# yangao07/LAMSA

Hardware: AMD Instinct MI355X
Metric: aligned Gbase/s, 10 kbp ONT-error reads (12%: sub/ins/del 4% each), -T ont2d vs GRCh37-sized stand-in; inputs resident in HBM when the timed region starts (upload excluded: see pcie_inclusive_*) (higher is better)
Workload: dtype int32

## Files before the change

### lamsa_amd/csrc/hp_core.h

```cpp
#pragma once
#include <hp/wave.h>
#include "../../include/lamsa_hp.h"

namespace hp {

typedef int32_t cig_t;
enum { C_M = 0, C_I = 1, C_D = 2, C_N = 3, C_S = 4, C_H = 5, C_EQ = 7, C_X = 8 };
enum { ST_OVERFLOW = LAMSA_HP_ST_OVERFLOW, ST_REFEXIT = LAMSA_HP_ST_REFEXIT, ST_UNSUPPORTED = LAMSA_HP_ST_UNSUPPORTED,
       ST_DEAD = ST_OVERFLOW | ST_REFEXIT | ST_UNSUPPORTED };

#define HP_NEG_INF (-0x40000000)

struct Arena {
    char *base; size_t cap, top;
};
HP_INL void arena_init(Arena &a, void *base, size_t cap) { a.base = (char *)base; a.cap = cap; a.top = 0; }
HP_INL size_t arena_mark(const Arena &a) { return a.top; }
HP_INL void arena_release(Arena &a, size_t m) { a.top = m; }

#ifndef HP_LDS_CELLS
#define HP_LDS_CELLS 512
#endif
#ifndef HP_LDS_Z_BYTES
#define HP_LDS_Z_BYTES 512
#endif
#define HP_LDS_WORDS (2 * HP_LDS_CELLS + HP_LDS_CELLS / 4 + HP_LDS_Z_BYTES / 4)
#ifndef HP_CHAIN_LDS_WORDS
#define HP_CHAIN_LDS_WORDS 2432
#endif
#define HP_BOTH_LDS_WORDS (HP_CHAIN_LDS_WORDS > HP_LDS_WORDS ? HP_CHAIN_LDS_WORDS : HP_LDS_WORDS)
#define HP_LANE_STRIP_WORDS HP_CHAIN_LDS_WORDS

struct Ctx {
    const lamsa_hp_para *P;
    HP_L int32_t *lds;
    int lds_words;
    Arena tmp;
    int status;
    long long n_cells;
    long long *prof;
    long long *prof_dp = nullptr;
    int lds_epoch;
};
#if defined(HP_PROF_EDGE) && (defined(HP_PROF_TRACK) || defined(HP_PROF_FILL))
#error "-DHP_PROF_EDGE, -DHP_PROF_TRACK and -DHP_PROF_FILL all use prof slots 16 .. 23: one of them per build"
#endif
#ifdef HP_PROF_FILL
#define HP_PROF_CHAIN_ON 0
#define HP_TADD_FILL(cx, slot, v) HP_TADD(cx, slot, v)
#else
#define HP_PROF_CHAIN_ON 1
#define HP_TADD_FILL(cx, slot, v) do { } while (0)
#endif
#ifdef HP_PROF
#define HP_T0(v) const long long v = wv::clock()
#define HP_TADD(cx, slot, v) do { if ((cx).prof) { (cx).prof[slot] += wv::clock() - (v); (cx).prof[(slot) + 1] += 1; } } while (0)
#else
#define HP_T0(v) do { } while (0)
#define HP_TADD(cx, slot, v) do { } while (0)
#endif

#ifndef HP_DPLOG
#define HP_DPLOG(kind, qlen, tlen, w, cells) do { } while (0)
#endif
#ifndef HP_STAT
#define HP_STAT(i) do { } while (0)
#endif
#ifndef HP_STAT_ADD
#define HP_STAT_ADD(i, n) ((void)0)
#endif
#ifndef HP_STAT_MAX
#define HP_STAT_MAX(i, v) ((void)0)
#endif
#ifdef HP_STAT_SLOTS
static_assert(HP_STAT_SLOTS >= 92, "the array of the path counters ends before the last slot the device sources use");
#define HP_STATX_ADD(i, n) HP_STAT_ADD(i, n)
#define HP_STATX_MAX(i, v) HP_STAT_MAX(i, v)
#else
#define HP_STATX_ADD(i, n) ((void)0)
#define HP_STATX_MAX(i, v) ((void)0)
#endif

HP_INL void *arena_alloc(Ctx &cx, size_t bytes) {
    size_t b = (bytes + 15) & ~(size_t)15;
    if (cx.tmp.top + b > cx.tmp.cap) { cx.status |= ST_OVERFLOW; return nullptr; }
    void *p = cx.tmp.base + cx.tmp.top;
    cx.tmp.top += b;
    return p;
}

struct CigV { cig_t *c; int n, cap; };
HP_INL void cig_bind(CigV &v, cig_t *mem, int cap) { v.c = mem; v.n = 0; v.cap = mem ? cap : 0; }
HP_INL bool cig_alloc(Ctx &cx, CigV &v, int cap) {
    cig_t *m = (cig_t *)arena_alloc(cx, (size_t)cap * sizeof(cig_t));
    cig_bind(v, m, cap);
    return m != nullptr;
}
HP_INL void cig_raw_push(Ctx &cx, CigV &v, cig_t w) {
    if (v.n >= v.cap) { cx.status |= ST_OVERFLOW; return; }
    v.c[v.n++] = w;
}
HP_INL void cig_push0(Ctx &cx, CigV &v, cig_t w) {
    if (v.n > 0 && (v.c[v.n - 1] & 0xf) == (w & 0xf)) { v.c[v.n - 1] += (w >> 4) << 4; return; }
    cig_raw_push(cx, v, w);
}
HP_INL void cig_push1(Ctx &cx, CigV &v, cig_t w) { if ((w >> 4) == 0) return; cig_push0(cx, v, w); }
HP_FN void cig_pushv(Ctx &cx, CigV &v, const cig_t *c, int n) {
    if (n == 0) return;
    const HP_G cig_t *src = (const HP_G cig_t *)c;
    HP_G cig_t *dst = (HP_G cig_t *)v.c;
    const int vn = v.n;
    int j = 0;
    if (vn > 0) {
        const cig_t last = dst[vn - 1], c0 = src[0];
        if ((last & 0xf) == (c0 & 0xf)) { dst[vn - 1] = last + ((c0 >> 4) << 4); j = 1; }
        else if (((last & 0xf) == C_I && (c0 & 0xf) == C_S) || ((last & 0xf) == C_S && (c0 & 0xf) == C_I)) {
            dst[vn - 1] = (((last >> 4) + (c0 >> 4)) << 4) | C_S; j = 1;
        }
    }
    const int m = n - j;
    if (vn + m > v.cap) { cx.status |= ST_OVERFLOW; return; }
    for (int b0 = 0; b0 < m; b0 += 64) { WAVE_FOR(l) { const int i = b0 + l; if (i < m) dst[vn + i] = src[j + i]; } }
    v.n = vn + m;
    wv::sync();
}
HP_FN void cig_pushw(Ctx &cx, CigV &v, cig_t w) {
    if (v.n > 0) {
        const cig_t last = v.c[v.n - 1];
        if ((last & 0xf) == (w & 0xf)) { v.c[v.n - 1] = last + ((w >> 4) << 4); return; }
        if (((last & 0xf) == C_I && (w & 0xf) == C_S) || ((last & 0xf) == C_S && (w & 0xf) == C_I)) { v.c[v.n - 1] = (((last >> 4) + (w >> 4)) << 4) | C_S; return; }
    }
    if (v.n + 1 > v.cap) { cx.status |= ST_OVERFLOW; return; }
    v.c[v.n++] = w;
}
HP_FN void cig_invert(cig_t *c, int n) {
    HP_G cig_t *g = (HP_G cig_t *)c;
    for (int b0 = 0; b0 < n / 2; b0 += 64) {
        WAVE_FOR(l) { const int a = b0 + l; if (a < n / 2) { const cig_t x = g[a], y = g[n - 1 - a]; g[a] = y; g[n - 1 - a] = x; } }
    }
    wv::sync();
}
HP_FN int cig_readlen(const cig_t *c, int n) {
    const HP_G cig_t *g = (const HP_G cig_t *)c;
    int tot = 0;
    for (int b0 = 0; b0 < n; b0 += 64) {
        wv::Lane<int> x;
        WAVE_FOR(l) { const int i = b0 + l; int v = 0; if (i < n) { const cig_t w = g[i]; const int op = w & 0xf; if (op == C_M || op == C_I || op == C_S) v = w >> 4; } x[l] = v; }
        tot += wv::reduce_sum(x);
    }
    return tot;
}
HP_FN int cig_reflen(const cig_t *c, int n) {
    const HP_G cig_t *g = (const HP_G cig_t *)c;
    int tot = 0;
    for (int b0 = 0; b0 < n; b0 += 64) {
        wv::Lane<int> x;
        WAVE_FOR(l) { const int i = b0 + l; int v = 0; if (i < n) { const cig_t w = g[i]; const int op = w & 0xf; if (op == C_M || op == C_D || op == C_H) v = w >> 4; } x[l] = v; }
        tot += wv::reduce_sum(x);
    }
    return tot;
}

struct Seq { const uint8_t *p; int stride; };
HP_INL int seq_at(const Seq &s, int i) { return s.p[(long)i * s.stride]; }
HP_INL Seq seq_fwd(const uint8_t *p) { Seq s; s.p = p; s.stride = 1; return s; }
HP_INL Seq seq_rev(const uint8_t *p, int len) { Seq s; s.p = p + (len > 0 ? len - 1 : 0); s.stride = -1; return s; }

HP_INL int sub_score(const lamsa_hp_para *P, int t, int q) { return (t > 3 || q > 3) ? -1 : (t == q ? P->match : -P->mis); }

HP_INL int iabs(int x) { return x < 0 ? -x : x; }
HP_INL int imin(int a, int b) { return a < b ? a : b; }
HP_INL int imax(int a, int b) { return a > b ? a : b; }

}
```

### lamsa_amd/csrc/hp_ksw.h

```cpp
#pragma once
#include "hp_core.h"

namespace hp {

#define HP_ZSTRIDE(n_col) ((((n_col) + 7) >> 3) << 2)
HP_INL size_t z_cap(const Ctx &cx) { const int w = cx.lds_words - (2 * HP_LDS_CELLS + HP_LDS_CELLS / 4); return w > 0 ? (size_t)w * 4 : 0; }
HP_INL size_t z_cap_pk(const Ctx &cx) { return cx.lds_words > 0 ? (size_t)cx.lds_words * 4 : 0; }
#define HP_ZFITS(n_col, rows) ((size_t)HP_ZSTRIDE(n_col) * (size_t)(rows) <= z_cap(cx))
HP_INL int z_nibble(int dir) { return (dir & 3) | ((dir >> 2) & 1) << 2 | ((dir >> 5) & 1) << 3; }
HP_INL void z_row_clear(HP_L uint8_t *LZ, int row, int n_col) {
    HP_L int *p = (HP_L int *)(LZ + row * HP_ZSTRIDE(n_col));
    const int nd = HP_ZSTRIDE(n_col) >> 2;
    for (int d0 = 0; d0 < nd; d0 += 64) { WAVE_FOR(l) { if (d0 + l < nd) p[d0 + l] = -1; } }
}
HP_INL void z_put(HP_L uint8_t *LZ, int row, int n_col, int c, int dir) {
    HP_L int *p = (HP_L int *)(LZ + row * HP_ZSTRIDE(n_col)) + (c >> 3);
    wv::lds_and(p, (int)~((unsigned)(~z_nibble(dir) & 0xf) << ((c & 7) << 2)));
}

HP_FN void dp_backtrack(Ctx &cx, const HP_L uint8_t *lz, const uint8_t *z, const int32_t *rowb, int n_col, int w, int i, int k, CigV &out, int pk_stride = 0)
{
    pk_stride = wv::uni(pk_stride);
    const bool in_lds = z == nullptr;
    const HP_G uint8_t *gz = (const HP_G uint8_t *)wv::uni64((long long)z);
// ... 551 lines not shown
            wv::scan_max_excl(key, HP_SCAN_IDENT);
            WAVE_FOR(l) {
                hcur[l] = -1;
                if (l >= beg && l < end) {
                    int f = 0 - (l - beg) * e_ins;
                    if (l > beg) { const int g = key[l] - (l - 1) * e_ins; f = g > f ? g : f; }
                    int M = m[l], ee = Es[l], h, tt;
                    int dir = M > ee ? 0 : 1; h = M > ee ? M : ee;
                    dir = h > f ? dir : 2;    h = h > f ? h : f;
                    tt = M - oe_del; tt = tt > 0 ? tt : 0; ee -= e_del;
                    if (ee > tt) dir |= 1 << 2; else ee = tt;
                    tt = M - oe_ins; tt = tt > 0 ? tt : 0; f -= e_ins;
                    if (f > tt) dir |= 2 << 4;
                    Es[l] = ee;
                    hcur[l] = h;
                    if (zl) z_put(LZ, i, n_col, l - d_beg, dir); else gz[(long)i * n_col + (l - d_beg)] = (uint8_t)dir;
                }
            }
            int mrow = 0, mj = -1;
            {
                const int hmax = wv::reduce_max(hcur);
                if (hmax >= 0) {
                    wv::Lane<int> eq;
                    WAVE_FOR(l) eq[l] = hcur[l] == hmax;
                    mrow = hmax; mj = 63 - __builtin_clzll(wv::ballot(eq));
                }
            }
            const int h_last = beg < end ? wv::bcast(hcur, end - 1) : h1_init;
            WAVE_FOR(l) { if (hcur[l] < 0) hcur[l] = 0; }
            wv::shr1(hcur, 0);
            wv::Lane<int> nz;
            WAVE_FOR(l) {
                if (beg < end) { if (l == beg) Hs[l] = h1_init; else if (l > beg && l <= end) Hs[l] = hcur[l]; }
                else if (l == end) Hs[l] = h1_init;
                if (l == end) Es[l] = 0;
                nz[l] = l >= beg && l <= end && (Hs[l] != 0 || Es[l] != 0);
            }
            const int jj = beg < end ? end : beg;
            if (jj == qlen) {
                max_ie = gscore > h_last ? max_ie : i;
                gscore = gscore > h_last ? gscore : h_last;
            }
            if (mrow == 0) { stop_rows = true; break; }
            if (mrow > max) { max = mrow; max_i = i; max_j = mj; }
            else if (zdrop > 0) {
                if (i - max_i > mj - max_j) { if (max - mrow - ((i - max_i) - (mj - max_j)) * e_del > zdrop) { stop_rows = true; break; } }
                else { if (max - mrow - ((mj - max_j) - (i - max_i)) * e_ins > zdrop) { stop_rows = true; break; } }
            }
            {
                const unsigned long long nzm = wv::ballot(nz);
                const unsigned long long lowm = nzm & (end < 64 ? ((1ull << end) - 1) : ~0ull);
                const int nb = lowm ? __builtin_ctzll(lowm) : end;
                const unsigned long long upm = nzm & ~((1ull << nb) - 1);
                const int jl = upm ? 63 - __builtin_clzll(upm) : nb - 1;
                beg = nb;
                end = jl + 2 < qlen ? jl + 2 : qlen;
            }
        }
    }
    int i, k;
    if (gscore <= 0 || gscore <= max - end_bonus) { i = max_i; k = max_j; }
    else { i = max_ie; k = qlen - 1; }
    er.qle = k + 1; er.tle = i + 1; er.score = max;
    if (out) { wv::sync(); HP_T0(tb0_); dp_backtrack(cx, zl ? LZ : nullptr, z, rowb, n_col, w, i, k, *out); HP_TADD(cx, 28, tb0_); }
    cx.n_cells += cells_;
    arena_release(cx.tmp, mark);
    HP_TADD(cx, 26, te0_);
#ifdef HP_PROF
    HP_TADD(cx, 60, te0_);
#endif
    return er;
}

#define HP_REGN_SETS 4
#define HP_REGN_QMAX(ns) (64 * (ns) - 2)
HP_INL unsigned long long lt_mask64(int x) { return x <= 0 ? 0ull : (x >= 64 ? ~0ull : ((1ull << x) - 1)); }
template <int NS>
HP_NOINL ExtRes ksw_extend_regn(Ctx &cx, int qlen, Seq q, int tlen, Seq t, int w, int h0, CigV *out)
{
    long long cells_ = 0;
    ExtRes er; er.score = 0; er.qle = 0; er.tle = 0;
    HP_T0(te0_);
    qlen = wv::uni(qlen); tlen = wv::uni(tlen); w = wv::uni(w); h0 = wv::uni(h0);
    const lamsa_hp_para *P = cx.P;
    const int o_ins = wv::uni(P->ins_ext_o), e_ins = wv::uni(P->ins_ext_e), o_del = wv::uni(P->del_ext_o), e_del = wv::uni(P->del_ext_e);
    const int end_bonus = wv::uni(P->end_bonus), zdrop = wv::uni(P->zdrop);
    const int oe_del = o_del + e_del, oe_ins = o_ins + e_ins;
    const int n_col = qlen < 2 * w + 1 ? qlen : 2 * w + 1;
    const size_t mark = arena_mark(cx.tmp);
    const bool zl = HP_ZFITS(n_col, tlen);
    uint8_t *z = zl ? nullptr : (uint8_t *)arena_alloc(cx, (size_t)n_col * tlen + 1);
    int32_t *rowb = zl ? nullptr : (int32_t *)arena_alloc(cx, sizeof(int32_t) * 2 * ((size_t)tlen + 1));
    if (!zl && (!z || !rowb)) { arena_release(cx.tmp, mark); return er; }
#ifdef HP_PROF
    if (!zl && cx.prof) { cx.prof[52] += (long long)n_col * tlen; cx.prof[53] += 1; }
#endif
    HP_L uint8_t *LZ = (HP_L uint8_t *)(cx.lds + 2 * HP_LDS_CELLS) + HP_LDS_CELLS;
    HP_G uint8_t *gz = (HP_G uint8_t *)wv::uni64((long long)z);
    HP_G int32_t *growb = (HP_G int32_t *)wv::uni64((long long)rowb);
    const int sc_match = wv::uni(P->match), sc_mis = -wv::uni(P->mis);
    const HP_G uint8_t *gq = (const HP_G uint8_t *)wv::uni64((long long)q.p); const int qs = wv::uni(q.stride);
    const HP_G uint8_t *gt = (const HP_G uint8_t *)wv::uni64((long long)t.p); const int ts = wv::uni(t.stride);
    const int h1v = h0 > oe_ins ? h0 - oe_ins : 0;
    wv::Lane<int> Hs[NS], Es[NS], hcur[NS], qbp, je0, tl;
    WAVE_FOR(l) { qbp[l] = 0; je0[l] = l * e_ins; tl[l] = 4; }
#pragma unroll
    for (int c = 0; c < NS; ++c) {
        WAVE_FOR(l) {
            const int j = 64 * c + l;
            Hs[c][l] = j == 0 ? h0 : (j == 1 ? h1v : ((j <= qlen && h1v - (j - 2) * e_ins > e_ins) ? h1v - (j - 1) * e_ins : 0));
            Es[c][l] = 0;
            qbp[l] |= (j < qlen ? (int)gq[(long)j * qs] : 4) << (3 * c);
        }
    }
    int max = h0, max_i = -1, max_j = -1, max_ie = -1, gscore = -1;
    int beg = 0, end = qlen;
    bool stop_rows = false;
    for (int ib = 0; ib < tlen && !stop_rows; ib += 64) {
        { WAVE_FOR(l) { const int ii = ib + l; tl[l] = ii < tlen ? gt[(long)ii * ts] : 4; } }
        const int ti_first = wv::bcast(tl, 0);
        const int ie = ib + 64 < tlen ? ib + 64 : tlen;
        for (int i = ib; i < ie; ++i) {
            const int ti = i == ib ? ti_first : wv::bcast(tl, i & 63);
            const int d_beg = i > w ? i - w : 0;
            if (beg < i - w) beg = i - w;
            if (end > i + w + 1) end = i + w + 1;
            if (end > qlen) end = qlen;
            cells_ += end > beg ? end - beg : 0;
            if (zl) { z_row_clear(LZ, i, n_col); wv::sync(); }
            else { growb[2 * i] = beg; growb[2 * i + 1] = end; }
            int h1_init;
            if (beg == 0) { h1_init = h0 - (o_del + e_del * (i + 1)); if (h1_init < 0) h1_init = 0; }
            else h1_init = 0;
            const int fbase = beg * e_ins;
            int carry = HP_SCAN_IDENT;
#pragma unroll
            for (int c = 0; c < NS; ++c) {
                const int jc = 64 * c * e_ins;
                wv::Lane<int> m, key;
                WAVE_FOR(l) {
                    const int j = 64 * c + l;
                    const int hm = Hs[c][l], qb = (qbp[l] >> (3 * c)) & 7;
                    const int M = hm ? hm + HP_SUB(ti, qb) : 0;
                    int tt = M - oe_ins; tt = tt > 0 ? tt : 0;
                    m[l] = M;
                    key[l] = (j >= beg && j < end) ? tt + je0[l] + jc : HP_SCAN_IDENT;
                }
                const int top = wv::scan_max_excl_top(key, HP_SCAN_IDENT);
                WAVE_FOR(l) {
                    const int j = 64 * c + l;
                    hcur[c][l] = -1;
                    if (j >= beg && j < end) {
                        const int je = je0[l] + jc;
                        int f = fbase - je;
                        if (j > beg) { const int kk = key[l] > carry ? key[l] : carry; const int g = kk - je + e_ins; f = g > f ? g : f; }
                        int M = m[l], ee = Es[c][l], h, tt;
                        int dir = M > ee ? 0 : 1; h = M > ee ? M : ee;
                        dir = h > f ? dir : 2;    h = h > f ? h : f;
                        tt = M - oe_del; tt = tt > 0 ? tt : 0; ee -= e_del;
                        if (ee > tt) dir |= 1 << 2; else ee = tt;
                        tt = M - oe_ins; tt = tt > 0 ? tt : 0; f -= e_ins;
                        if (f > tt) dir |= 2 << 4;
                        Es[c][l] = ee;
                        hcur[c][l] = h;
                        if (zl) z_put(LZ, i, n_col, j - d_beg, dir); else gz[(long)i * n_col + (j - d_beg)] = (uint8_t)dir;
                    }
                }
                carry = top > carry ? top : carry;
            }
            int mrow = 0, mj = -1;
            {
                wv::Lane<int> hm;
                WAVE_FOR(l) {
                    int v = hcur[0][l];
#pragma unroll
                    for (int c = 1; c < NS; ++c) v = hcur[c][l] > v ? hcur[c][l] : v;
                    hm[l] = v;
                }
                const int hmax = wv::reduce_max(hm);
                if (hmax >= 0) {
                    mrow = hmax;
                    bool got = false;
#pragma unroll
                    for (int c = NS - 1; c >= 0; --c) {
                        if (got) continue;
                        wv::Lane<int> eq;
                        WAVE_FOR(l) eq[l] = hcur[c][l] == hmax;
                        const unsigned long long b = wv::ballot(eq);
                        if (b) { mj = 64 * c + 63 - __builtin_clzll(b); got = true; }
                    }
                }
            }
            int h_last = h1_init;
            if (beg < end) {
#pragma unroll
                for (int c = 0; c < NS; ++c) if (((end - 1) >> 6) == c) h_last = wv::bcast(hcur[c], (end - 1) & 63);
            }
#pragma unroll
            for (int c = 0; c < NS; ++c) { WAVE_FOR(l) { if (hcur[c][l] < 0) hcur[c][l] = 0; } }
#pragma unroll
            for (int c = NS - 1; c >= 0; --c) {
                const int below = c > 0 ? wv::bcast(hcur[c > 0 ? c - 1 : 0], 63) : 0;
                wv::shr1(hcur[c], below);
            }
            unsigned long long nzm[NS];
#pragma unroll
            for (int c = 0; c < NS; ++c) {
                wv::Lane<int> nz;
                WAVE_FOR(l) {
                    const int j = 64 * c + l;
                    if (beg < end) { if (j == beg) Hs[c][l] = h1_init; else if (j > beg && j <= end) Hs[c][l] = hcur[c][l]; }
                    else if (j == end) Hs[c][l] = h1_init;
                    if (j == end) Es[c][l] = 0;
                    nz[l] = j >= beg && j <= end && (Hs[c][l] != 0 || Es[c][l] != 0);
                }
                nzm[c] = wv::ballot(nz);
            }
            const int jj = beg < end ? end : beg;
            if (jj == qlen) {
                max_ie = gscore > h_last ? max_ie : i;
                gscore = gscore > h_last ? gscore : h_last;
            }
            if (mrow == 0) { stop_rows = true; break; }
            if (mrow > max) { max = mrow; max_i = i; max_j = mj; }
            else if (zdrop > 0) {
                if (i - max_i > mj - max_j) { if (max - mrow - ((i - max_i) - (mj - max_j)) * e_del > zdrop) { stop_rows = true; break; } }
                else { if (max - mrow - ((mj - max_j) - (i - max_i)) * e_ins > zdrop) { stop_rows = true; break; } }
            }
            {
                const int e_set = end >> 6;
                const unsigned long long e_bit = 1ull << (end & 63);
                bool end_nz = false, got = false;
                int nb = end, jl = -1;
#pragma unroll
                for (int c = 0; c < NS; ++c) {
                    unsigned long long lo = nzm[c];
                    if (c == e_set) { end_nz = lo & e_bit; lo &= ~e_bit; }
                    if (!got && lo) { nb = 64 * c + __builtin_ctzll(lo); got = true; }
                }
                if (got) {
                    bool gl = false;
#pragma unroll
                    for (int c = NS - 1; c >= 0; --c) if (!gl && nzm[c]) { jl = 64 * c + 63 - __builtin_clzll(nzm[c]); gl = true; }
                } else jl = end_nz ? end : end - 1;
                beg = nb;
                end = jl + 2 < qlen ? jl + 2 : qlen;
            }
        }
    }
    int i, k;
    if (gscore <= 0 || gscore <= max - end_bonus) { i = max_i; k = max_j; }
    else { i = max_ie; k = qlen - 1; }
    er.qle = k + 1; er.tle = i + 1; er.score = max;
    if (out) { wv::sync(); HP_T0(tb0_); dp_backtrack(cx, zl ? LZ : nullptr, z, rowb, n_col, w, i, k, *out); HP_TADD(cx, 28, tb0_); }
    cx.n_cells += cells_;
    arena_release(cx.tmp, mark);
    HP_TADD(cx, 26, te0_);
    return er;
}

#define HP_PK_QMAX(ns) (128 * (ns) - 2)
#ifndef HP_PK_RT
#define HP_PK_RT 1
#endif
#define HP_PK_IDENT (-16000)
#ifdef HP_PROF
#define HP_PD2_T0(v) const long long v = wv::clock()
#define HP_PD2_ADD(cx, on, slot, v) do { if ((cx).prof_dp && (on)) (cx).prof_dp[slot] += wv::clock() - (v); } while (0)
#define HP_PD2_CLASS(qlen, w) (pkb_sets_q(qlen, w) == 2 && (qlen) + 3 <= 256)
#else
#define HP_PD2_T0(v) do { } while (0)
#define HP_PD2_ADD(cx, on, slot, v) do { } while (0)
#endif

HP_INL int pkb_sets_q(int qlen, int w)
{
    for (int ns = 1; ns <= 4; ns *= 2) if (2 * w + 3 + 18 * ns <= 128 * ns || qlen + 3 <= 128 * ns) return ns;
    return 0;
}
HP_INL bool pkb_extend_ok(const lamsa_hp_para *P, int qlen, int h0, int ns)
{
    const int mx = P->match > P->mis ? P->match : P->mis;
    const int pen = (P->ins_ext_o > P->del_ext_o ? P->ins_ext_o : P->del_ext_o) + (P->ins_ext_e > P->del_ext_e ? P->ins_ext_e : P->del_ext_e);
    const int ext = P->ins_ext_e > P->del_ext_e ? P->ins_ext_e : P->del_ext_e;
    return ns > 0 && mx > 0 && mx < 256 && pen >= 0 && pen < 4000 && P->ins_ext_e >= 0 && P->del_ext_e >= 0 && P->ins_ext_o >= 0 && P->del_ext_o >= 0 &&
           (long long)h0 + (long long)qlen * mx < 23000 && (long long)(128 * ns + 2) * ext < 8000 && qlen + 128 * ns < 32000;
}
HP_INL int pkb_key_lo(int h, int j)
{
#if defined(__HIP_DEVICE_COMPILE__)
    return (int)__builtin_amdgcn_perm((unsigned)h, (unsigned)j, 0x05040100u);
#else
    return (int)(((unsigned)h << 16) | ((unsigned)j & 0xffffu));
#endif
}
HP_INL int pkb_key_hi(int h, int j)
{
#if defined(__HIP_DEVICE_COMPILE__)
    return (int)__builtin_amdgcn_perm((unsigned)h, (unsigned)j, 0x07060302u);
#else
    return (int)(((unsigned)h & 0xffff0000u) | ((unsigned)j >> 16));
#endif
}
template <int NS, bool FIXED>
HP_NOINL ExtRes ksw_extend_band(Ctx &cx, int qlen, Seq q, int tlen, Seq t, int w, int h0, CigV *out)
{
    long long cells_ = 0;
    ExtRes er; er.score = 0; er.qle = 0; er.tle = 0;
    HP_T0(te0_);
    qlen = wv::uni(qlen); tlen = wv::uni(tlen); w = wv::uni(w); h0 = wv::uni(h0);
    HP_PD2_T0(tp0_);
    const lamsa_hp_para *P = cx.P;
    const int o_ins = wv::uni(P->ins_ext_o), e_ins = wv::uni(P->ins_ext_e), o_del = wv::uni(P->del_ext_o), e_del = wv::uni(P->del_ext_e);
    const int end_bonus = wv::uni(P->end_bonus), zdrop = wv::uni(P->zdrop);
    const int oe_del = o_del + e_del, oe_ins = o_ins + e_ins;
    const int n_col = qlen < 2 * w + 1 ? qlen : 2 * w + 1;
    constexpr bool KEY0 = FIXED && NS < 4, KEEP_JRE = NS < 4;
    constexpr int LC = 2 * NS, WN = 128 * NS, zs = 64 * NS;
    const size_t mark = arena_mark(cx.tmp);
    uint8_t *z = (uint8_t *)arena_alloc(cx, (size_t)zs * tlen + 16);
    int32_t *rowb = (int32_t *)arena_alloc(cx, sizeof(int32_t) * 2 * ((size_t)tlen + 1));
    if (!z || !rowb) { arena_release(cx.tmp, mark); return er; }
#ifdef HP_PROF
    if (cx.prof) { cx.prof[52] += (long long)zs * tlen; cx.prof[53] += 1; }
#endif
    HP_G uint8_t *gz = (HP_G uint8_t *)wv::uni64((long long)z);
    HP_G int32_t *growb = (HP_G int32_t *)wv::uni64((long long)rowb);
    const int sc_match = wv::uni(P->match), sc_mis = -wv::uni(P->mis);
    const HP_G uint8_t *gq = (const HP_G uint8_t *)wv::uni64((long long)q.p); const int qs = wv::uni(q.stride);
    const HP_G uint8_t *gt = (const HP_G uint8_t *)wv::uni64((long long)t.p); const int ts = wv::uni(t.stride);
    const int h1v = h0 > oe_ins ? h0 - oe_ins : 0;
    const int OEI = pk::rep(oe_ins), OED = pk::rep(oe_del), EI = pk::rep(e_ins), ED = pk::rep(e_del);
    const int DSC = pk::rep(sc_match - sc_mis), MIS = pk::rep(sc_mis), IDENT = pk::rep(HP_PK_IDENT);
#define HP_PKB_EH0(j) ((j) == 0 ? h0 : ((j) == 1 ? h1v : (((j) <= qlen && h1v - ((j) - 2) * e_ins > e_ins) ? h1v - ((j) - 1) * e_ins : 0)))
#define HP_PKB_LOAD(jb_) do { \
        _Pragma("unroll") for (int r_ = 0; r_ < NS; ++r_) { \
            int hv_[2], oh_ = 0, nn_ = 0; \
            _Pragma("unroll") for (int b_ = 0; b_ < 2; ++b_) { \
                const int j_ = (jb_) + 2 * r_ + b_; \
                hv_[b_] = HP_PKB_EH0(j_); \
                const int code_ = j_ < qlen ? (int)gq[(long)j_ * qs] : 4; \
                if (code_ < 4) oh_ |= 1 << (code_ + 16 * b_); else nn_ |= (int)(0xffffu << (16 * b_)); \
            } \
            Hs[r_][l] = pk::pack(hv_[0], hv_[1]); Es[r_][l] = 0; qoh[r_][l] = oh_; qN[r_][l] = nn_; \
        } \
        JB[l] = pk::pack(jb_, (jb_) + 1); } while (0)
    wv::Lane<int> Hs[NS], Es[NS], qoh[NS], qN[NS], hcur[NS], M[NS], INB[NS], JRE[NS], pre[NS], JB, tl;
    WAVE_FOR(l) { tl[l] = 4; HP_PKB_LOAD(LC * l); }
    if constexpr (FIXED) HP_STAT(16);
    if constexpr (KEY0) {
        WAVE_FOR(l) {
#pragma unroll
            for (int r = 0; r < NS; ++r) JRE[r][l] = pk::mul(pk::add(JB[l], pk::rep(2 * r)), EI);
        }
    }
    int top = WN; (void)top;
    int max = h0, max_i = -1, max_j = -1, max_ie = -1, gscore = -1;
    int beg = 0, end = qlen;
    bool stop_rows = false;
    HP_PD2_ADD(cx, NS == 2 && qlen + 3 <= WN, 44, tp0_);
    HP_PD2_T0(tp1_);
    for (int ib = 0; ib < tlen && !stop_rows; ib += 64) {
        { WAVE_FOR(l) { const int ii = ib + l; tl[l] = ii < tlen ? gt[(long)ii * ts] : 4; } }
        const int ti_first = wv::bcast(tl, 0);
        const int ie = ib + 64 < tlen ? ib + 64 : tlen;
        for (int i = ib; i < ie; ++i) {
            const int ti = i == ib ? ti_first : wv::bcast(tl, i & 63);
            if (beg < i - w) beg = i - w;
            if (end > i + w + 1) end = i + w + 1;
            if (end > qlen) end = qlen;
            cells_ += end > beg ? end - beg : 0;
            { WAVE_FOR(l) { if (l < 2) growb[2 * i + l] = l ? end : beg; } }
            int h1_init;
            if (beg == 0) { h1_init = h0 - (o_del + e_del * (i + 1)); if (h1_init < 0) h1_init = 0; }
            else h1_init = 0;
            if (beg >= end) {
                if (beg == qlen) { max_ie = gscore > h1_init ? max_ie : i; gscore = gscore > h1_init ? gscore : h1_init; }
                stop_rows = true; break;
            }
            if (!FIXED && end + 3 > top) {
                const int lr = (top / LC) & 63;
                WAVE_FOR(l) { const int d = (l - lr) & 63; if (d < 8) { const int jb = top + d * LC; HP_PKB_LOAD(jb); } }
                top += 8 * LC;
            }
            const int tsh = ti & 3, tN = ti > 3 ? -1 : 0;
            const int BEG = pk::rep(beg), END = pk::rep(end), H1 = pk::rep(h1_init);
            const int l0 = FIXED ? 0 : (beg / LC) & 63;
            const int F0 = KEY0 ? pk::rep(beg * e_ins) : 0;
            wv::Lane<int> ka, kb;
            WAVE_FOR(l) {
                int run = HP_PK_IDENT;
#pragma unroll
                for (int r = 0; r < NS; ++r) {
                    const int jp = pk::add(JB[l], pk::rep(2 * r));
                    const int in = pk::neg_mask(pk::sub(jp, END)) & ~pk::neg_mask(pk::sub(jp, BEG));
                    const int eq = (qoh[r][l] >> tsh) & 0x00010001;
                    const int S = pk::add(pk::mul(eq, DSC), MIS) | qN[r][l] | tN;
                    const int hm = Hs[r][l];
                    const int m = pk::mul(pk::add(hm, S), pk::min_u(hm, 0x00010001));
                    const int t1 = pk::max(pk::sub(m, OEI), 0);
                    const int jre = KEY0 ? JRE[r][l] : pk::mul(pk::sub(jp, BEG), EI);
                    const int k = pk::sel(in, pk::add(t1, jre), IDENT);
                    const int klo = pk::lo(k), khi = pk::hi(k);
                    const int p0 = run; run = run > klo ? run : klo;
                    const int p1 = run; run = run > khi ? run : khi;
                    M[r][l] = m; INB[r][l] = in; if constexpr (!KEY0 && KEEP_JRE) JRE[r][l] = jre; pre[r][l] = pk::pack(p0, p1);
                }
                if constexpr (FIXED) { ka[l] = run; kb[l] = HP_PK_IDENT; }
                else { ka[l] = l >= l0 ? run : HP_PK_IDENT; kb[l] = l < l0 ? run : HP_PK_IDENT; }
            }
            int topA = HP_PK_IDENT;
            if constexpr (FIXED) wv::scan_max_excl(ka, HP_PK_IDENT);
            else { topA = wv::scan_max_excl_top(ka, HP_PK_IDENT); wv::scan_max_excl(kb, HP_PK_IDENT); }
            wv::Lane<int> best;
            WAVE_FOR(l) {
                const int pl = FIXED ? ka[l] : (l >= l0 ? ka[l] : (topA > kb[l] ? topA : kb[l]));
                const int PP = pk::rep(pl);
                int zw = 0, bk = -1;
#pragma unroll
                for (int r = 0; r < NS; ++r) {
                    const int jp = pk::add(JB[l], pk::rep(2 * r));
                    const int jre = KEEP_JRE ? JRE[r][l] : pk::mul(pk::sub(jp, BEG), EI);
                    const int in = INB[r][l], m = M[r][l];
                    const int pr = pk::max(pre[r][l], PP);
                    int f = pk::max(pk::add(pk::sub(pr, jre), EI), pk::sub(F0, jre));
                    const int tI = pk::max(pk::sub(m, OEI), 0);
                    int ee = Es[r][l];
                    const int m1 = pk::neg_mask(pk::sub(ee, m));
                    int h = pk::max(m, ee);
                    const int m2 = pk::neg_mask(pk::sub(f, h));
                    int d = pk::sel(m2, ~m1 & 0x00010001, 0x00020002);
                    h = pk::max(h, f);
                    const int tD = pk::max(pk::sub(m, OED), 0);
                    ee = pk::sub(ee, ED);
                    d |= pk::neg_mask(pk::sub(tD, ee)) & 0x00040004;
                    ee = pk::max(ee, tD);
                    f = pk::sub(f, EI);
                    d |= pk::neg_mask(pk::sub(tI, f)) & 0x00080008;
                    Es[r][l] = pk::sel(in, ee, Es[r][l]);
                    const int hc = pk::sel(in, h, -1);
                    hcur[r][l] = hc;
                    zw |= ((d | (d >> 12)) & 0xff) << (8 * r);
                    const int k0 = pkb_key_lo(hc, jp), k1 = pkb_key_hi(hc, jp);
                    bk = bk > k0 ? bk : k0; bk = bk > k1 ? bk : k1;
                }
                best[l] = bk;
                if constexpr (NS == 1) gz[(long)i * zs + l] = (uint8_t)zw;
                else if constexpr (NS == 2) *(HP_G uint16_t *)(gz + (long)i * zs + 2 * l) = (uint16_t)zw;
                else *(HP_G uint32_t *)(gz + (long)i * zs + 4 * l) = (uint32_t)zw;
            }
            int mrow = 0, mj = -1;
            { const int b = wv::reduce_max(best); if (b >= 0) { mrow = b >> 16; mj = b & 0xffff; } }
            wv::Lane<int> rot = hcur[NS - 1], LB;
            wv::ror1(rot);
            WAVE_FOR(l) {
                int bits = 0;
#pragma unroll
                for (int r = 0; r < NS; ++r) {
                    const int below = r > 0 ? hcur[r > 0 ? r - 1 : 0][l] : rot[l];
                    const int hsh = pk::shift_up(hcur[r][l], below);
                    const int in = INB[r][l];
                    const int upd = ~pk::neg_mask(hsh);
                    int hs = Hs[r][l], es = Es[r][l];
                    hs = pk::sel(upd, hsh, hs);
                    hs = pk::sel(in & ~upd, H1, hs);
                    es &= ~(upd & ~in);
                    Hs[r][l] = hs; Es[r][l] = es;
                    const int nzh = pk::min_u((hs | es) & (in | upd), 0x00010001);
                    bits |= ((nzh | (nzh >> 15)) & 3) << (2 * r);
                }
                LB[l] = bits;
            }
            if (end == qlen) {
                const int le = FIXED ? (end - 1) / LC : ((end - 1) / LC) & 63, sl = (end - 1) % LC;
                int v = 0;
#pragma unroll
                for (int r = 0; r < NS; ++r) if ((sl >> 1) == r) v = wv::bcast(hcur[r], le);
                const int h_last = (sl & 1) ? pk::hi(v) : pk::lo(v);
                max_ie = gscore > h_last ? max_ie : i;
                gscore = gscore > h_last ? gscore : h_last;
            }
            if (mrow == 0) { stop_rows = true; break; }
            if (mrow > max) { max = mrow; max_i = i; max_j = mj; }
            else if (zdrop > 0) {
                if (i - max_i > mj - max_j) { if (max - mrow - ((i - max_i) - (mj - max_j)) * e_del > zdrop) { stop_rows = true; break; } }
                else { if (max - mrow - ((mj - max_j) - (i - max_i)) * e_ins > zdrop) { stop_rows = true; break; } }
            }
            {
                const unsigned long long any = wv::ballot(LB);
                int nb = end, jl = end - 1;
                if (any) {
                    const unsigned long long rt = l0 ? ((any >> l0) | (any << (64 - l0))) : any;
                    const int df = __builtin_ctzll(rt), dl = 63 - __builtin_clzll(rt);
                    const int bf = wv::bcast(LB, FIXED ? df : (l0 + df) & 63), bl = wv::bcast(LB, FIXED ? dl : (l0 + dl) & 63);
                    const int bb = FIXED ? 0 : beg / LC;
                    const int jf = (bb + df) * LC + __builtin_ctz((unsigned)bf), jx = (bb + dl) * LC + (31 - __builtin_clz((unsigned)bl));
                    if (jf < end) nb = jf;
                    jl = jx;
                }
                beg = nb;
                end = jl + 2 < qlen ? jl + 2 : qlen;
            }
        }
    }
#undef HP_PKB_LOAD
#undef HP_PKB_EH0
    int i, k;
    if (gscore <= 0 || gscore <= max - end_bonus) { i = max_i; k = max_j; }
    else { i = max_ie; k = qlen - 1; }
    er.qle = k + 1; er.tle = i + 1; er.score = max;
    HP_PD2_ADD(cx, NS == 2 && qlen + 3 <= WN, 45, tp1_);
    HP_PD2_T0(tp2_);
    if (out) { wv::sync(); HP_T0(tb0_); dp_backtrack(cx, nullptr, z, rowb, n_col, w, i, k, *out, zs); HP_TADD(cx, 28, tb0_); }
    HP_PD2_ADD(cx, NS == 2 && qlen + 3 <= WN, 46, tp2_);
    cx.n_cells += cells_;
    arena_release(cx.tmp, mark);
    HP_TADD(cx, 26, te0_);
    return er;
}

#define HP_PKG_NEG (-12000)
#define HP_PKG_IDENT (-24000)
HP_INL bool pk_global_ok(const lamsa_hp_para *P, int qlen, int tlen, int o_del, int e_del, int o_ins, int e_ins)
{
    const int mx = P->match > P->mis ? P->match : P->mis;
    const long long o = o_del > o_ins ? o_del : o_ins, e = e_del > e_ins ? e_del : e_ins;
    return mx > 0 && mx < 256 && o_del >= 0 && e_del >= 0 && o_ins >= 0 && e_ins >= 0 && o + e * ((long long)qlen + tlen + 4) + (long long)mx * (qlen + 2) < 4000;
}
template <int NS>
HP_NOINL int ksw_global_pk(Ctx &cx, int qlen, Seq q, int tlen, Seq t, int o_del, int e_del, int o_ins, int e_ins, int w, CigV *out)
{
    long long cells_ = 0;
    HP_T0(tg0_);
    qlen = wv::uni(qlen); tlen = wv::uni(tlen); w = wv::uni(w);
    o_del = wv::uni(o_del); e_del = wv::uni(e_del); o_ins = wv::uni(o_ins); e_ins = wv::uni(e_ins);
    const int oe_del = o_del + e_del, oe_ins = o_ins + e_ins;
    const int n_col = qlen < 2 * w + 1 ? qlen : 2 * w + 1;
    const int zs = 64 * NS;
    const size_t mark = arena_mark(cx.tmp);
    const bool zl = (size_t)zs * (size_t)tlen <= z_cap_pk(cx);
    if (out && zl) ++cx.lds_epoch;
    uint8_t *z = (out && !zl) ? (uint8_t *)arena_alloc(cx, (size_t)zs * tlen + 1) : nullptr;
    if (out && !zl && !z) { arena_release(cx.tmp, mark); return 0; }
    HP_L uint8_t *LZ = (HP_L uint8_t *)cx.lds;
    HP_G uint8_t *gz = (HP_G uint8_t *)wv::uni64((long long)z);
    const int sc_match = wv::uni(cx.P->match), sc_mis = -wv::uni(cx.P->mis);
    const HP_G uint8_t *gq = (const HP_G uint8_t *)wv::uni64((long long)q.p); const int qs = wv::uni(q.stride);
    const HP_G uint8_t *gt = (const HP_G uint8_t *)wv::uni64((long long)t.p); const int ts = wv::uni(t.stride);
    const int OEI = pk::rep(oe_ins), OED = pk::rep(oe_del), EI = pk::rep(e_ins), ED = pk::rep(e_del);
    const int DSC = pk::rep(sc_match - sc_mis), MIS = pk::rep(sc_mis), IDENT = pk::rep(HP_PKG_IDENT), NEG = pk::rep(HP_PKG_NEG);
    wv::Lane<int> Hs[NS], Es[NS], qoh[NS], qN[NS], hcur[NS], jp0, jep0, tl;
    WAVE_FOR(l) { jp0[l] = pk::pack(2 * l, 2 * l + 1); jep0[l] = pk::pack(2 * l * e_ins, (2 * l + 1) * e_ins); tl[l] = 4; }
#pragma unroll
    for (int c = 0; c < NS; ++c) {
        WAVE_FOR(l) {
            int hv[2], oh = 0, nn = 0;
#pragma unroll
            for (int b = 0; b < 2; ++b) {
                const int j = 128 * c + 2 * l + b;
                hv[b] = j == 0 ? 0 : (j <= w ? -(o_ins + e_ins * j) : HP_PKG_NEG);
                const int code = j < qlen ? (int)gq[(long)j * qs] : 4;
                if (code < 4) oh |= 1 << (code + 16 * b); else nn |= (int)(0xffffu << (16 * b));
            }
            Hs[c][l] = pk::pack(hv[0], hv[1]); Es[c][l] = NEG;
            qoh[c][l] = oh; qN[c][l] = nn;
        }
    }
    for (int ib = 0; ib < tlen; ib += 64) {
        { WAVE_FOR(l) { const int ii = ib + l; tl[l] = ii < tlen ? gt[(long)ii * ts] : 4; } }
        const int ti_first = wv::bcast(tl, 0);
        const int ie = ib + 64 < tlen ? ib + 64 : tlen;
        for (int i = ib; i < ie; ++i) {
            const int ti = i == ib ? ti_first : wv::bcast(tl, i & 63);
            const int beg = i > w ? i - w : 0;
            const int end = i + w + 1 < qlen ? i + w + 1 : qlen;
            cells_ += end > beg ? end - beg : 0;
            const int h1_init = beg == 0 ? -(o_del + e_del * (i + 1)) : HP_PKG_NEG;
            const int tsh = ti & 3, tN = ti > 3 ? -1 : 0;
            const int BEG = pk::rep(beg), END = pk::rep(end), FB = pk::rep(HP_PKG_NEG + beg * e_ins), H1 = pk::rep(h1_init);
            int carry = HP_PKG_IDENT;
            wv::Lane<int> inb[NS];
#pragma unroll
            for (int c = 0; c < NS; ++c) {
                wv::Lane<int> key, klo, M;
                WAVE_FOR(l) {
                    const int jp = pk::add(jp0[l], pk::rep(128 * c));
                    inb[c][l] = pk::neg_mask(pk::sub(jp, END)) & ~pk::neg_mask(pk::sub(jp, BEG));
                    const int eq = (qoh[c][l] >> tsh) & 0x00010001;
                    const int S = pk::add(pk::mul(eq, DSC), MIS) | qN[c][l] | tN;
                    const int m = pk::add(Hs[c][l], S);
                    const int jep = pk::add(jep0[l], pk::rep(128 * c * e_ins));
                    const int k = pk::sel(inb[c][l], pk::add(pk::sub(m, OEI), jep), IDENT);
                    M[l] = m;
                    klo[l] = pk::lo(k);
                    const int kh = pk::hi(k);
                    key[l] = klo[l] > kh ? klo[l] : kh;
                }
                const int top = wv::scan_max_excl_top(key, HP_PKG_IDENT);
                WAVE_FOR(l) {
                    const int jep = pk::add(jep0[l], pk::rep(128 * c * e_ins));
                    const int s0 = key[l] > carry ? key[l] : carry, s1 = s0 > klo[l] ? s0 : klo[l];
                    const int pre = pk::pack(s0, s1);
                    int f = pk::max(pk::add(pk::sub(pre, jep), EI), pk::sub(FB, jep));
                    const int m = M[l];
                    int ee = Es[c][l];
                    int d = pk::neg_mask(pk::sub(m, ee)) & 0x00010001;
                    int h = pk::max(m, ee);
                    d = pk::sel(pk::neg_mask(pk::sub(h, f)), 0x00020002, d);
                    h = pk::max(h, f);
                    const int tD = pk::sub(m, OED);
                    ee = pk::sub(ee, ED);
                    d |= pk::neg_mask(pk::sub(tD, ee)) & 0x00040004;
                    ee = pk::max(ee, tD);
                    f = pk::sub(f, EI);
                    d |= pk::neg_mask(pk::sub(pk::sub(m, OEI), f)) & 0x00080008;
                    const int in = inb[c][l];
                    Es[c][l] = pk::sel(in, ee, Es[c][l]);
                    hcur[c][l] = h;
                    if (out && zl) LZ[i * zs + 64 * c + l] = (uint8_t)((d | (d >> 12)) & 0xff);
                    else if (out && in) gz[(long)i * zs + 64 * c + l] = (uint8_t)((d | (d >> 12)) & 0xff);
                }
                carry = top > carry ? top : carry;
            }
#pragma unroll
            for (int c = NS - 1; c >= 0; --c) {
                const int below = c > 0 ? wv::bcast(hcur[c > 0 ? c - 1 : 0], 63) : 0, below_in = c > 0 ? wv::bcast(inb[c > 0 ? c - 1 : 0], 63) : 0;
                wv::Lane<int> dn = hcur[c], dm = inb[c];
                wv::shr1(dn, below); wv::shr1(dm, below_in);
                WAVE_FOR(l) {
                    const int hsh = pk::shift_up(hcur[c][l], dn[l]), upd = pk::shift_up(inb[c][l], dm[l]);
                    const int in = inb[c][l];
                    int hs = pk::sel(upd, hsh, Hs[c][l]);
                    hs = pk::sel(in & ~upd, H1, hs);
                    Hs[c][l] = hs;
                    Es[c][l] = pk::sel(upd & ~in, NEG, Es[c][l]);
                }
            }
        }
    }
    int score = 0;
#pragma unroll
    for (int c = 0; c < NS; ++c) if ((qlen >> 7) == c) { const int v = wv::bcast(Hs[c], (qlen >> 1) & 63); score = (qlen & 1) ? pk::hi(v) : pk::lo(v); }
    if (score <= HP_PKG_NEG / 2) score = HP_NEG_INF + (score - HP_PKG_NEG);
    if (out) {
        const int i = tlen - 1;
        const int k = (i + w + 1 < qlen ? i + w + 1 : qlen) - 1;
        wv::sync();
        HP_T0(tb0_);
        dp_backtrack(cx, zl ? LZ : nullptr, z, nullptr, n_col, w, i, k, *out, zs);
        HP_TADD(cx, 28, tb0_);
    }
    cx.n_cells += cells_;
    arena_release(cx.tmp, mark);
    HP_TADD(cx, 24, tg0_);
    return score;
}

HP_INL int ksw_global(Ctx &cx, int qlen, Seq q, int tlen, Seq t,
                      int o_del, int e_del, int o_ins, int e_ins, int w, CigV *out)
{
    if (out) out->n = 0;
    if (qlen < 0 || tlen < 0) { cx.status |= ST_REFEXIT; return 0; }
    { const int d = iabs(qlen - tlen) + 3; if (w < d) w = d; }
    HP_DPLOG(1, qlen, tlen, w, 0);
    if (qlen <= HP_REG_QMAX) return ksw_global_reg(cx, qlen, q, tlen, t, o_del, e_del, o_ins, e_ins, w, out);
    if (HP_PK_RT && qlen <= HP_PK_QMAX(2) && pk_global_ok(cx.P, qlen, tlen, o_del, e_del, o_ins, e_ins)) {
        HP_STAT(18);
        return qlen <= HP_PK_QMAX(1) ? ksw_global_pk<1>(cx, qlen, q, tlen, t, o_del, e_del, o_ins, e_ins, w, out) : ksw_global_pk<2>(cx, qlen, q, tlen, t, o_del, e_del, o_ins, e_ins, w, out);
    }
    HP_STAT(19);
    if (2 * w + 4 + 64 <= HP_LDS_CELLS) return ksw_global_lds(cx, qlen, q, tlen, t, o_del, e_del, o_ins, e_ins, w, out);
    return ksw_global_wide(cx, qlen, q, tlen, t, o_del, e_del, o_ins, e_ins, w, out);
}

HP_NOINL ExtRes ksw_extend_lds(Ctx &cx, int qlen, Seq q, int tlen, Seq t, int w, int h0, CigV *out)
{
    ++cx.lds_epoch;
    long long cells_ = 0;
    ExtRes er; er.score = 0; er.qle = 0; er.tle = 0;
    HP_T0(te0_);
    qlen = wv::uni(qlen); tlen = wv::uni(tlen); w = wv::uni(w); h0 = wv::uni(h0);
    const lamsa_hp_para *P = cx.P;
    const int o_ins = wv::uni(P->ins_ext_o), e_ins = wv::uni(P->ins_ext_e), o_del = wv::uni(P->del_ext_o), e_del = wv::uni(P->del_ext_e);
    const int end_bonus = wv::uni(P->end_bonus), zdrop = wv::uni(P->zdrop);
    const int oe_del = o_del + e_del, oe_ins = o_ins + e_ins;
    const int n_col = qlen < 2 * w + 1 ? qlen : 2 * w + 1;
    const size_t mark = arena_mark(cx.tmp);
    const bool zl = HP_ZFITS(n_col, tlen);
    uint8_t *z = zl ? nullptr : (uint8_t *)arena_alloc(cx, (size_t)n_col * tlen + 1);
    int32_t *rowb = zl ? nullptr : (int32_t *)arena_alloc(cx, sizeof(int32_t) * 2 * ((size_t)tlen + 1));
    if (!zl && (!z || !rowb)) { arena_release(cx.tmp, mark); return er; }
#ifdef HP_PROF
    if (!zl && cx.prof) { cx.prof[52] += (long long)n_col * tlen; cx.prof[53] += 1; }
#endif
    HP_L int32_t *LH = cx.lds, *LE = cx.lds + HP_LDS_CELLS;
    HP_L uint8_t *LQ = (HP_L uint8_t *)(cx.lds + 2 * HP_LDS_CELLS), *LZ = LQ + HP_LDS_CELLS;
    HP_G uint8_t *gz = (HP_G uint8_t *)wv::uni64((long long)z);
    HP_G int32_t *growb = (HP_G int32_t *)wv::uni64((long long)rowb);
    const int sc_match = wv::uni(P->match), sc_mis = -wv::uni(P->mis);
    const HP_G uint8_t *gq = (const HP_G uint8_t *)wv::uni64((long long)q.p); const int qs = wv::uni(q.stride);
    const HP_G uint8_t *gt = (const HP_G uint8_t *)wv::uni64((long long)t.p); const int ts = wv::uni(t.stride);
    const int h1v = h0 > oe_ins ? h0 - oe_ins : 0;
#define HP_EH0(j) ((j) == 0 ? h0 : ((j) == 1 ? h1v : (((j) <= qlen && h1v - ((j) - 2) * e_ins > e_ins) ? h1v - ((j) - 1) * e_ins : 0)))
    int hw = -1, qw = -1;
    wv::Lane<int> tl;
    WAVE_FOR(l) { tl[l] = 4; }
    int max = h0, max_i = -1, max_j = -1, max_ie = -1, gscore = -1;
    int beg = 0, end = qlen;
    bool stop_rows = false;
    for (int ib = 0; ib < tlen && !stop_rows; ib += 64) {
    { WAVE_FOR(l) { const int ii = ib + l; tl[l] = ii < tlen ? gt[(long)ii * ts] : 4; } }
    const int ti_first = wv::bcast(tl, 0);
    const int ie = ib + 64 < tlen ? ib + 64 : tlen;
    for (int i = ib; i < ie; ++i) {
        const int ti = i == ib ? ti_first : wv::bcast(tl, i & 63);
        const int d_beg = i > w ? i - w : 0;
        if (beg < i - w) beg = i - w;
        if (end > i + w + 1) end = i + w + 1;
        if (end > qlen) end = qlen;
        cells_ += end > beg ? end - beg : 0;
        if (end > hw) {
            for (int j0 = hw + 1; j0 <= end; j0 += 64) { WAVE_FOR(l) { const int j = j0 + l; if (j <= end) { LH[j & HP_LDS_MASK] = HP_EH0(j); LE[j & HP_LDS_MASK] = 0; } } }
            hw = end;
        }
        while (end - 1 > qw) { WAVE_FOR(l) { const int j = qw + 1 + l; if (j < qlen) LQ[j & HP_LDS_MASK] = gq[(long)j * qs]; } qw += 64; }
        if (zl) z_row_clear(LZ, i, n_col);
        else { growb[2 * i] = beg; growb[2 * i + 1] = end; }
        wv::sync();
        int h1_init;
        if (beg == 0) { h1_init = h0 - (o_del + e_del * (i + 1)); if (h1_init < 0) h1_init = 0; }
        else h1_init = 0;
        int carryH = wv::uni(LH[beg & HP_LDS_MASK]);
        int Fin = 0;
        long long best = -1;
        int h_last = h1_init;
        int first_nz = -1, last_nz = -1, prev_h_nz = h1_init != 0;
        wv::sync();
        if (beg < end) LH[beg & HP_LDS_MASK] = h1_init; else LH[end & HP_LDS_MASK] = h1_init;
        for (int j0 = beg; j0 < end; j0 += 64) {
            const int nxt = j0 + 64;
            const int carry_next = wv::uni(LH[nxt & HP_LDS_MASK]);
            wv::Lane<int> m, e, key;
            WAVE_FOR(l) {
                const int j = j0 + l;
                if (j < end) {
                    const int hm = l == 0 ? carryH : LH[j & HP_LDS_MASK];
                    const int qb = LQ[j & HP_LDS_MASK];
                    const int M = hm ? hm + HP_SUB(ti, qb) : 0;
                    int tt = M - oe_ins; tt = tt > 0 ? tt : 0;
                    m[l] = M; e[l] = LE[j & HP_LDS_MASK]; key[l] = tt + j * e_ins;
                } else { m[l] = 0; e[l] = 0; key[l] = HP_SCAN_IDENT; }
            }
            wv::scan_max_excl(key, HP_SCAN_IDENT);
            wv::sync();
            wv::Lane<int> fnext, hnz, enz, hh;
            WAVE_FOR(l) {
                const int j = j0 + l;
                fnext[l] = 0; hnz[l] = 0; enz[l] = 0; hh[l] = -1;
                if (j < end) {
                    int f = Fin - l * e_ins;
                    if (l > 0) { const int g = key[l] - (j - 1) * e_ins; f = g > f ? g : f; }
                    int M = m[l], ee = e[l], h, tt;
                    int dir = M > ee ? 0 : 1; h = M > ee ? M : ee;
                    dir = h > f ? dir : 2;    h = h > f ? h : f;
                    tt = M - oe_del; tt = tt > 0 ? tt : 0; ee -= e_del;
                    if (ee > tt) dir |= 1 << 2; else ee = tt;
                    tt = M - oe_ins; tt = tt > 0 ? tt : 0; f -= e_ins;
                    if (f > tt) dir |= 2 << 4; else f = tt;
                    LE[j & HP_LDS_MASK] = ee;
                    LH[(j + 1) & HP_LDS_MASK] = h;
                    if (zl) z_put(LZ, i, n_col, j - d_beg, dir); else gz[(long)i * n_col + (j - d_beg)] = (uint8_t)dir;
                    fnext[l] = f; hnz[l] = h != 0; enz[l] = ee != 0;
                    hh[l] = h;
                }
            }
            Fin = wv::bcast(fnext, 63);
            carryH = carry_next;
            {
                const int hmax = wv::reduce_max(hh);
                if (hmax >= 0) {
                    wv::Lane<int> eq;
                    WAVE_FOR(l) eq[l] = hh[l] == hmax;
                    const long long b = ((long long)hmax << 32) | (unsigned)(j0 + 63 - __builtin_clzll(wv::ballot(eq)));
                    if (b > best) best = b;
                }
                const int cnt = end - j0 < 64 ? end - j0 : 64;
                const unsigned long long bh = wv::ballot(hnz), be = wv::ballot(enz);
                const unsigned long long nzm = be | (bh << 1) | (unsigned long long)(prev_h_nz ? 1 : 0);
                const unsigned long long inrow = cnt == 64 ? ~0ull : ((1ull << cnt) - 1);
                if (first_nz < 0 && (nzm & inrow)) first_nz = j0 + __builtin_ctzll(nzm & inrow);
                if (nzm & inrow) last_nz = j0 + 63 - __builtin_clzll(nzm & inrow);
                prev_h_nz = (int)((bh >> (cnt - 1)) & 1);
            }
        }
        wv::sync();
        if (beg < end) h_last = wv::uni(LH[end & HP_LDS_MASK]);
        LE[end & HP_LDS_MASK] = 0;
        if (end > hw) hw = end;
        const int jj = beg < end ? end : beg;
        if (jj == qlen) {
            max_ie = gscore > h_last ? max_ie : i;
            gscore = gscore > h_last ? gscore : h_last;
        }
        int mrow = 0, mj = -1;
        if (best >= 0) { mrow = (int)(best >> 32); mj = (int)(best & 0xffffffffll); }
        if (mrow == 0) { stop_rows = true; break; }
// ... 183 lines not shown
```

Measured before the change: 4.267.

## Rebase sliding band window by lane rotation instead of wrapped ring indexing

In the non-fixed banded extension, the ring-buffer layout (wrap offset l0, a split max-scan into ka/kb, and rotated ballots) is replaced. When the band outgrows the 64-lane window, the per-lane H/E/query state is shifted down with gathers and the window base advances, so every row can use a single plain prefix-max scan and unrotated ballot decoding. Per-row band begin/end values are collected into lane registers with v_writelane and written once per 64-row block, instead of a global store on every row. The shift costs several gathers per rebase and needs per-lane z offsets. The row max now comes from scan_max_excl_top instead of reduce_max, and extra stat slots are added.

```diff
diff --git a/lamsa_amd/csrc/hp_core.h b/lamsa_amd/csrc/hp_core.h
--- a/lamsa_amd/csrc/hp_core.h
+++ b/lamsa_amd/csrc/hp_core.h
@@ -73,7 +73,7 @@
 #define HP_STAT_MAX(i, v) ((void)0)
 #endif
 #ifdef HP_STAT_SLOTS
-static_assert(HP_STAT_SLOTS >= 92, "the array of the path counters ends before the last slot the device sources use");
+static_assert(HP_STAT_SLOTS >= 97, "the array of the path counters ends before the last slot the device sources use");
 #define HP_STATX_ADD(i, n) HP_STAT_ADD(i, n)
 #define HP_STATX_MAX(i, v) HP_STAT_MAX(i, v)
 #else
diff --git a/lamsa_amd/csrc/hp_ksw.h b/lamsa_amd/csrc/hp_ksw.h
--- a/lamsa_amd/csrc/hp_ksw.h
+++ b/lamsa_amd/csrc/hp_ksw.h
@@ -877,6 +877,16 @@
     return (int)(((unsigned)h & 0xffff0000u) | ((unsigned)j >> 16));
 #endif
 }
+HP_INL void pkb_putlane2(wv::Lane<int> &a, wv::Lane<int> &b, int dst, int va, int vb)
+{
+#if defined(__HIP_DEVICE_COMPILE__)
+    int keep;
+    asm("s_mov_b32 %2, m0\n\ts_mov_b32 m0, %5\n\tv_writelane_b32 %0, %3, m0\n\tv_writelane_b32 %1, %4, m0\n\ts_mov_b32 m0, %2"
+        : "+v"(a.v), "+v"(b.v), "=&s"(keep) : "s"(va), "s"(vb), "s"(dst));
+#else
+    wv::setlane(a, dst, va); wv::setlane(b, dst, vb);
+#endif
+}
 template <int NS, bool FIXED>
 HP_NOINL ExtRes ksw_extend_band(Ctx &cx, int qlen, Seq q, int tlen, Seq t, int w, int h0, CigV *out)
 {
@@ -890,7 +900,8 @@
     const int end_bonus = wv::uni(P->end_bonus), zdrop = wv::uni(P->zdrop);
     const int oe_del = o_del + e_del, oe_ins = o_ins + e_ins;
     const int n_col = qlen < 2 * w + 1 ? qlen : 2 * w + 1;
-    constexpr bool KEY0 = FIXED && NS < 4, KEEP_JRE = NS < 4;
+    constexpr bool KEY0 = NS < 4;
+    constexpr bool LIM_LANES = NS < 4;
     constexpr int LC = 2 * NS, WN = 128 * NS, zs = 64 * NS;
     const size_t mark = arena_mark(cx.tmp);
     uint8_t *z = (uint8_t *)arena_alloc(cx, (size_t)zs * tlen + 16);
@@ -920,8 +931,8 @@
             Hs[r_][l] = pk::pack(hv_[0], hv_[1]); Es[r_][l] = 0; qoh[r_][l] = oh_; qN[r_][l] = nn_; \
         } \
         JB[l] = pk::pack(jb_, (jb_) + 1); } while (0)
-    wv::Lane<int> Hs[NS], Es[NS], qoh[NS], qN[NS], hcur[NS], M[NS], INB[NS], JRE[NS], pre[NS], JB, tl;
-    WAVE_FOR(l) { tl[l] = 4; HP_PKB_LOAD(LC * l); }
+    wv::Lane<int> Hs[NS], Es[NS], qoh[NS], qN[NS], hcur[NS], M[NS], INB[NS], JRE[NS], pre[NS], JB, tl, zoff, RB, RE;
+    WAVE_FOR(l) { tl[l] = 4; HP_PKB_LOAD(LC * l); zoff[l] = NS * l; RB[l] = 0; RE[l] = 0; }
     if constexpr (FIXED) HP_STAT(16);
     if constexpr (KEY0) {
         WAVE_FOR(l) {
@@ -929,7 +940,7 @@
             for (int r = 0; r < NS; ++r) JRE[r][l] = pk::mul(pk::add(JB[l], pk::rep(2 * r)), EI);
         }
     }
-    int top = WN; (void)top;
+    int base = 0; (void)base;
     int max = h0, max_i = -1, max_j = -1, max_ie = -1, gscore = -1;
     int beg = 0, end = qlen;
     bool stop_rows = false;
@@ -939,13 +950,15 @@
         { WAVE_FOR(l) { const int ii = ib + l; tl[l] = ii < tlen ? gt[(long)ii * ts] : 4; } }
         const int ti_first = wv::bcast(tl, 0);
         const int ie = ib + 64 < tlen ? ib + 64 : tlen;
+        int n_lim = 0; (void)n_lim;
         for (int i = ib; i < ie; ++i) {
             const int ti = i == ib ? ti_first : wv::bcast(tl, i & 63);
             if (beg < i - w) beg = i - w;
             if (end > i + w + 1) end = i + w + 1;
             if (end > qlen) end = qlen;
             cells_ += end > beg ? end - beg : 0;
-            { WAVE_FOR(l) { if (l < 2) growb[2 * i + l] = l ? end : beg; } }
+            if constexpr (LIM_LANES) { pkb_putlane2(RB, RE, i & 63, beg, end); n_lim = i - ib + 1; }
+            else { WAVE_FOR(l) { if (l < 2) growb[2 * i + l] = l ? end : beg; } }
             int h1_init;
             if (beg == 0) { h1_init = h0 - (o_del + e_del * (i + 1)); if (h1_init < 0) h1_init = 0; }
             else h1_init = 0;
@@ -953,16 +966,27 @@
                 if (beg == qlen) { max_ie = gscore > h1_init ? max_ie : i; gscore = gscore > h1_init ? gscore : h1_init; }
                 stop_rows = true; break;
             }
-            if (!FIXED && end + 3 > top) {
-                const int lr = (top / LC) & 63;
-                WAVE_FOR(l) { const int d = (l - lr) & 63; if (d < 8) { const int jb = top + d * LC; HP_PKB_LOAD(jb); } }
-                top += 8 * LC;
+            if constexpr (!FIXED) {
+                if (end + 3 > base + WN) {
+                    const int s = (beg - base) / LC;
+                    HP_STATX_ADD(92, 1); HP_STATX_MAX(93, s); HP_STATX_MAX(94, 64 - s); HP_STATX_ADD(95, i == ib ? 1 : 0); HP_STATX_ADD(96, (i & 63) == 63 ? 1 : 0);
+                    base += s * LC;
+                    wv::Lane<int> from;
+                    WAVE_FOR(l) from[l] = (l + s) & 63;
+#pragma unroll
+                    for (int r = 0; r < NS; ++r) { Hs[r] = wv::gather(Hs[r], from); Es[r] = wv::gather(Es[r], from); qoh[r] = wv::gather(qoh[r], from); qN[r] = wv::gather(qN[r], from); }
+                    WAVE_FOR(l) {
+                        const int jb = base + LC * l;
+                        if (l >= 64 - s) HP_PKB_LOAD(jb);
+                        JB[l] = pk::pack(jb, jb + 1);
+                        zoff[l] = ((base / LC + l) & 63) * NS;
+                    }
+                }
             }
             const int tsh = ti & 3, tN = ti > 3 ? -1 : 0;
             const int BEG = pk::rep(beg), END = pk::rep(end), H1 = pk::rep(h1_init);
-            const int l0 = FIXED ? 0 : (beg / LC) & 63;
-            const int F0 = KEY0 ? pk::rep(beg * e_ins) : 0;
-            wv::Lane<int> ka, kb;
+            const int F0 = KEY0 ? pk::rep((beg - base) * e_ins) : 0;
+            wv::Lane<int> ka;
             WAVE_FOR(l) {
                 int run = HP_PK_IDENT;
 #pragma unroll
@@ -979,23 +1003,19 @@
                     const int klo = pk::lo(k), khi = pk::hi(k);
                     const int p0 = run; run = run > klo ? run : klo;
                     const int p1 = run; run = run > khi ? run : khi;
-                    M[r][l] = m; INB[r][l] = in; if constexpr (!KEY0 && KEEP_JRE) JRE[r][l] = jre; pre[r][l] = pk::pack(p0, p1);
-                }
-                if constexpr (FIXED) { ka[l] = run; kb[l] = HP_PK_IDENT; }
-                else { ka[l] = l >= l0 ? run : HP_PK_IDENT; kb[l] = l < l0 ? run : HP_PK_IDENT; }
-            }
-            int topA = HP_PK_IDENT;
-            if constexpr (FIXED) wv::scan_max_excl(ka, HP_PK_IDENT);
-            else { topA = wv::scan_max_excl_top(ka, HP_PK_IDENT); wv::scan_max_excl(kb, HP_PK_IDENT); }
+                    M[r][l] = m; INB[r][l] = in; pre[r][l] = pk::pack(p0, p1);
+                }
+                ka[l] = run;
+            }
+            wv::scan_max_excl(ka, HP_PK_IDENT);
             wv::Lane<int> best;
             WAVE_FOR(l) {
-                const int pl = FIXED ? ka[l] : (l >= l0 ? ka[l] : (topA > kb[l] ? topA : kb[l]));
-                const int PP = pk::rep(pl);
+                const int PP = pk::rep(ka[l]);
                 int zw = 0, bk = -1;
 #pragma unroll
                 for (int r = 0; r < NS; ++r) {
                     const int jp = pk::add(JB[l], pk::rep(2 * r));
-                    const int jre = KEEP_JRE ? JRE[r][l] : pk::mul(pk::sub(jp, BEG), EI);
+                    const int jre = KEY0 ? JRE[r][l] : pk::mul(pk::sub(jp, BEG), EI);
                     const int in = INB[r][l], m = M[r][l];
                     const int pr = pk::max(pre[r][l], PP);
                     int f = pk::max(pk::add(pk::sub(pr, jre), EI), pk::sub(F0, jre));
@@ -1020,12 +1040,13 @@
                     bk = bk > k0 ? bk : k0; bk = bk > k1 ? bk : k1;
                 }
                 best[l] = bk;
-                if constexpr (NS == 1) gz[(long)i * zs + l] = (uint8_t)zw;
-                else if constexpr (NS == 2) *(HP_G uint16_t *)(gz + (long)i * zs + 2 * l) = (uint16_t)zw;
-                else *(HP_G uint32_t *)(gz + (long)i * zs + 4 * l) = (uint32_t)zw;
+                const int zo = FIXED ? NS * l : zoff[l];
+                if constexpr (NS == 1) gz[(long)i * zs + zo] = (uint8_t)zw;
+                else if constexpr (NS == 2) *(HP_G uint16_t *)(gz + (long)i * zs + zo) = (uint16_t)zw;
+                else *(HP_G uint32_t *)(gz + (long)i * zs + zo) = (uint32_t)zw;
             }
             int mrow = 0, mj = -1;
-            { const int b = wv::reduce_max(best); if (b >= 0) { mrow = b >> 16; mj = b & 0xffff; } }
+            { const int b = wv::scan_max_excl_top(best, -1); if (b >= 0) { mrow = b >> 16; mj = b & 0xffff; } }
             wv::Lane<int> rot = hcur[NS - 1], LB;
             wv::ror1(rot);
             WAVE_FOR(l) {
@@ -1047,7 +1068,7 @@
                 LB[l] = bits;
             }
             if (end == qlen) {
-                const int le = FIXED ? (end - 1) / LC : ((end - 1) / LC) & 63, sl = (end - 1) % LC;
+                const int le = (end - 1 - base) / LC, sl = (end - 1) % LC;
                 int v = 0;
 #pragma unroll
                 for (int r = 0; r < NS; ++r) if ((sl >> 1) == r) v = wv::bcast(hcur[r], le);
@@ -1065,11 +1086,9 @@
                 const unsigned long long any = wv::ballot(LB);
                 int nb = end, jl = end - 1;
                 if (any) {
-                    const unsigned long long rt = l0 ? ((any >> l0) | (any << (64 - l0))) : any;
-                    const int df = __builtin_ctzll(rt), dl = 63 - __builtin_clzll(rt);
-                    const int bf = wv::bcast(LB, FIXED ? df : (l0 + df) & 63), bl = wv::bcast(LB, FIXED ? dl : (l0 + dl) & 63);
-                    const int bb = FIXED ? 0 : beg / LC;
-                    const int jf = (bb + df) * LC + __builtin_ctz((unsigned)bf), jx = (bb + dl) * LC + (31 - __builtin_clz((unsigned)bl));
+                    const int df = __builtin_ctzll(any), dl = 63 - __builtin_clzll(any);
+                    const int bf = wv::bcast(LB, df), bl = wv::bcast(LB, dl);
+                    const int jf = base + df * LC + __builtin_ctz((unsigned)bf), jx = base + dl * LC + (31 - __builtin_clz((unsigned)bl));
                     if (jf < end) nb = jf;
                     jl = jx;
                 }
@@ -1077,6 +1096,7 @@
                 end = jl + 2 < qlen ? jl + 2 : qlen;
             }
         }
+        if constexpr (LIM_LANES) WAVE_FOR(l) { if (l < n_lim) { hp_v2i be; be.x = RB[l]; be.y = RE[l]; *(HP_G hp_v2i *)(growb + 2 * (ib + l)) = be; } }
     }
 #undef HP_PKB_LOAD
 #undef HP_PKB_EH0
```

Measured after the change: 4.317, median of 6. +1.2%, better.
